# DeltaPavonis/cpp_raytracer

Hardware: AMD Instinct MI355X
Metric: Msamples/sec + achieved HBM GB/s, RTOW final scene at 1/2/4/8 MI355X (higher is better)
Workload: dtype f64; 1 GPU; rtow_final seed 42, 1200x800, 500 spp, max_depth 50 (BASELINE config 2); primitives=485, bvh_nodes=115, partition=whole frame on one GPU

## Files before the change

cpp_raytracer_amd/csrc/crt_device.hip:

```cpp
#include <hip/hip_runtime.h>

#define CRT_HD __host__ __device__ __forceinline__

#include <algorithm>
#include <atomic>
#include <cmath>
#include <cstdio>
#include <cstring>
#include <limits>
#include <string>
#include <mutex>
#include <thread>
#include <type_traits>
#include <vector>

#include "crt_internal.h"
#include "crt_hip_util.h"
#include "crt_rows.h"
#include "crt_ray_class.h"
#include "crt_schlick.h"

#pragma clang fp contract(off)

namespace crt {

namespace dev {

#ifndef CRT_BLOCK
#define CRT_BLOCK 256
#endif
constexpr int kBlock = CRT_BLOCK;
#ifndef CRT_TILE_W
#define CRT_TILE_W 16
#endif
constexpr uint32_t kTileW = CRT_TILE_W, kTileH = 64 / CRT_TILE_W;
constexpr int kManyWaves = 5;
#ifndef CRT_PAIR_WALK
#define CRT_PAIR_WALK 1
#endif
constexpr double kScale = 1 / static_cast<double>(4294967295u - 1);

typedef double Dvec2 __attribute__((ext_vector_type(2)));
typedef uint32_t Uvec4 __attribute__((ext_vector_type(4)));

struct SceneView {
    const DevNode* nodes;
    const DevNodeF* fnodes;
    uint32_t ntop;
    const uint32_t* refs;
    const DevSphere* spheres;
    const DevSpherePair* spair;
    uint32_t spair_lds;
    const uint32_t* sphere_mat;
    const DevQuad* quads;
    const uint32_t* quad_mat;
    const DevMaterial* mats;
    const DevQuadF* quadf;
    const DevMaterial* sphere_mrec;
    const DevMaterial* quad_mrec;
    uint32_t quadf_lds;
    const DevQuadBox* quadbox;
    uint32_t refs_lds, spheres_lds, quads_lds;
    uint32_t inv64_lds;
    unsigned long long* guard;
    const uint16_t* links;
    uint32_t links_lds;
    uint32_t sentinel;
};

struct CamView {
    double o[3], p00[3], pdx[3], pdy[3], ddx[3], ddy[3];
    double defocus_angle;
    double bg[3];
    double t_min;
    double inv_spp;
    uint32_t w, h, spp, max_depth, base_seed;
};

struct Work {
    uint32_t owned_rows;
    uint32_t row_block, tile_count, tile_index;
    uint32_t col0, k0, bw, bh;
    uint32_t tiles_x, tiles_y, tiles;
    uint32_t chunks, chunk_len;
    uint32_t s0;
    uint32_t* queue;
    uint32_t segments;
    uint32_t n_items, bulk_items;
    uint32_t item_chunks, groups, bulk_chunks, tail_chunks;
    uint32_t rb_shift;
    uint32_t lds_nodes, lds_refs, lds_spheres, lds_quads, lds_quadf, lds_stack;
    uint32_t bytes_nodes, bytes_refs, bytes_spheres, bytes_quads, bytes_quadf;
    uint32_t lds_sph64, bytes_sph64;
    uint32_t sphere_only;
    uint32_t exact_slab;
    uint32_t ntop;
    uint32_t sentinel;
    uint32_t lds_cam;
    uint32_t lds_acc;
    uint32_t lds_inv64;
    uint32_t lds_links, bytes_links;
    uint32_t packed;
// ... 93 lines not shown
    h = fma(h, e, h);
    double d = fma(-g, g, x);
    g = fma(d, h, g);
    d = fma(-g, g, x);
    return fma(d, h, g);
}

template <bool FAST>
__device__ __forceinline__ double sqrt_exact(double x) {
    if (FAST) return sqrt_from_rsq(x, __builtin_amdgcn_rsq(x));
    return sqrt(x);
}
__device__ __forceinline__ double recip_core(double s) {
    double y = __builtin_amdgcn_rcp(s);
    y = fma(y, fma(-s, y, 1.0), y);
    y = fma(y, fma(-s, y, 1.0), y);
    return fma(fma(-s, y, 1.0), y, y);
}
template <bool FAST>
__device__ __forceinline__ double recip_exact(double s) {
    if (!FAST) return 1 / s;
    if (__builtin_expect(!(fabs(s) >= 0x1p-500 && fabs(s) <= 0x1p500), 0)) return 1 / s;
    return recip_core(s);
}

template <bool FAST = false>
__device__ __forceinline__ void random_unit_vector(uint32_t& s, double& x, double& y, double& z) {
    double m2;
    do {
        x = rnd_pm1(s);
        y = rnd_pm1(s);
        z = rnd_pm1(s);
        m2 = x * x + y * y + z * z;
    } while (!(m2 < 1));
    double inv = recip_exact<FAST>(sqrt_exact<FAST>(x * x + y * y + z * z));
    x = x * inv;
    y = y * inv;
    z = z * inv;
}

struct NodeRegs {
    double b[6];
    uint32_t index, count, axis, flags;
};

__device__ __forceinline__ NodeRegs load_node(const DevNode* nodes, uint32_t i) {
    const uint4* p = reinterpret_cast<const uint4*>(nodes + i);
    const uint4 q0 = p[0], q1 = p[1], q2 = p[2], q3 = p[3];
    NodeRegs n;
    n.b[0] = __hiloint2double(q0.y, q0.x);
    n.b[1] = __hiloint2double(q0.w, q0.z);
    n.b[2] = __hiloint2double(q1.y, q1.x);
    n.b[3] = __hiloint2double(q1.w, q1.z);
    n.b[4] = __hiloint2double(q2.y, q2.x);
    n.b[5] = __hiloint2double(q2.w, q2.z);
    n.index = q3.x;
    n.count = q3.y;
    n.axis = q3.z;
    n.flags = q3.w;
    return n;
}

__device__ __forceinline__ bool slab(const NodeRegs& n, const double o[3], const double inv[3],
                                     uint32_t neg, double tmin, double tmax) {
    const double bx0 = (neg & 1u) ? n.b[1] : n.b[0], bx1 = (neg & 1u) ? n.b[0] : n.b[1];
    const double by0 = (neg & 2u) ? n.b[3] : n.b[2], by1 = (neg & 2u) ? n.b[2] : n.b[3];
    const double bz0 = (neg & 4u) ? n.b[5] : n.b[4], bz1 = (neg & 4u) ? n.b[4] : n.b[5];
    double xtmin = (bx0 - o[0]) * inv[0];
    double xtmax = (bx1 - o[0]) * inv[0];
    const double ytmin = (by0 - o[1]) * inv[1];
    const double ytmax = (by1 - o[1]) * inv[1];
    const double ztmin = (bz0 - o[2]) * inv[2];
    const double ztmax = (bz1 - o[2]) * inv[2];
    const bool c1 = !(xtmin > ytmax || ytmin > xtmax);
    if (ytmin > xtmin) xtmin = ytmin;
    if (ytmax < xtmax) xtmax = ytmax;
    const bool c2 = !(xtmin > ztmax || ztmin > xtmax);
    if (ztmin > xtmin) xtmin = ztmin;
    if (ztmax < xtmax) xtmax = ztmax;
    return c1 & c2 & (xtmin < tmax) & (xtmax > tmin);
}

template <bool FAST = false>
__device__ __forceinline__ double recip_a(double a) {
    return (a >= 0x1p-500 && a <= 0x1p500) ? (FAST ? recip_core(a) : 1 / a) : __builtin_nan("");
}

__device__ __forceinline__ double div_a(double n, double a, double ia) {
    const double an = fabs(n);
    if (__builtin_expect(!(an >= 0x1p-500 && an <= 0x1p500 && ia == ia), 0)) return n / a;
    double q = n * ia;
    q = fma(fma(-a, q, n), ia, q);
    return fma(fma(-a, q, n), ia, q);
}

__device__ __forceinline__ double lim_tmax(double tmax, double a) { return tmax * a * (1 + 0x1p-30); }
__device__ __forceinline__ double lim_tmin(double tmin, double a) { return tmin * a * (1 - 0x1p-30); }

template <bool COARSE = true>
__device__ __forceinline__ bool hit_sphere(const DevSphere& sp, const double o[3], const double d[3],
                                           double a, double ia, double tmin, double tmax, double lo,
                                           double hi, double& t) {
    double ocx = o[0] - sp.c[0], ocy = o[1] - sp.c[1], ocz = o[2] - sp.c[2];
    double b = d[0] * ocx + d[1] * ocy + d[2] * ocz;
    double c = (ocx * ocx + ocy * ocy + ocz * ocz) - sp.r * sp.r;
    double disc = b * b - a * c;
    if (disc < 0) return false;
    const double rs = __builtin_amdgcn_rsq(disc);
    if (COARSE) {
        const double sqa = disc * rs;
        const double m = (fabs(b) + sqa) * 0x1p-12;
        const bool beyond = (-b - sqa) - m > hi;
        const bool before = (-b + sqa) + m < lo;
        if (beyond || before) return false;
    }
    double sq = sqrt_from_rsq(disc, rs);
    double root = div_a(-b - sq, a, ia);
    if (!(tmin < root && root < tmax)) {
        root = div_a(-b + sq, a, ia);
        if (!(tmin < root && root < tmax)) return false;
    }
    t = root;
    return true;
}

__device__ __forceinline__ float vmin(float a, float b) { float r; asm("v_min_f32 %0, %1, %2" : "=v"(r) : "v"(a), "v"(b)); return r; }
__device__ __forceinline__ float vmax(float a, float b) { float r; asm("v_max_f32 %0, %1, %2" : "=v"(r) : "v"(a), "v"(b)); return r; }
__device__ __forceinline__ float vmin3(float a, float b, float c) {
    float r;
    asm("v_min3_f32 %0, %1, %2, %3" : "=v"(r) : "v"(a), "v"(b), "v"(c));
    return r;
}
__device__ __forceinline__ float vmax_s(float a, float b) { float r; asm("v_max_f32 %0, %2, %1" : "=v"(r) : "v"(a), "s"(b)); return r; }
__device__ __forceinline__ float vmax_abs(float a, float b) {
    float r;
    asm("v_max_f32 %0, |%1|, |%2|" : "=v"(r) : "v"(a), "v"(b));
    return r;
}
__device__ __forceinline__ float vmax3_0(float a, float b) {
    float r;
    asm("v_max3_f32 %0, %1, %2, 0" : "=v"(r) : "v"(a), "v"(b));
    return r;
}
__device__ __forceinline__ float vmax3(float a, float b, float c) {
    float r;
    asm("v_max3_f32 %0, %1, %2, %3" : "=v"(r) : "v"(a), "v"(b), "v"(c));
    return r;
}

struct DevMinMax {
    static __device__ __forceinline__ float min(float a, float b) { return vmin(a, b); }
    static __device__ __forceinline__ float max(float a, float b) { return vmax(a, b); }
    static __device__ __forceinline__ float min3(float a, float b, float c) { return vmin3(a, b, c); }
    static __device__ __forceinline__ float max3(float a, float b, float c) { return vmax3(a, b, c); }
    static __device__ __forceinline__ float max_s(float a, float b) { return vmax_s(a, b); }
    static __device__ __forceinline__ float max_abs(float a, float b) { return vmax_abs(a, b); }
};

typedef float F2 __attribute__((ext_vector_type(2)));
struct LeafRay32 {
    F2 oxy, ozdx, dydz, akap, hilo;
};
__device__ __forceinline__ void leaf_ray32(const double o[3], const double d[3], double a, double tmin,
                                           double tmax, LeafRay32& L) {
    float o32[3];
    double e2 = 0;
#pragma unroll
    for (int k = 0; k < 3; ++k) {
        o32[k] = static_cast<float>(o[k]);
        const double e = o[k] - static_cast<double>(o32[k]);
        e2 = e2 + e * e;
    }
    L.oxy = F2{o32[0], o32[1]};
    L.ozdx = F2{o32[2], static_cast<float>(d[0])};
    L.dydz = F2{static_cast<float>(d[1]), static_cast<float>(d[2])};
    L.akap = F2{static_cast<float>(a), static_cast<float>(e2 * 0x1p22 + 0x1p-50)};
    L.hilo = F2{static_cast<float>(tmax * a * (1 + 0x1p-20)), static_cast<float>(tmin * a * (1 - 0x1p-20))};
}
__device__ __forceinline__ bool leaf_ray32_ok(const double o[3], const double d[3], double a) {
    bool ok = a >= 0x1p-60 && a <= 0x1p60;
#pragma unroll
    for (int k = 0; k < 3; ++k) ok = ok && fabs(o[k]) <= 0x1p30 && fabs(d[k]) <= 0x1p30;
    return ok;
}
__device__ __forceinline__ float vmul_abs(float a, float b) {
    float r;
    asm("v_mul_f32 %0, %1, |%2|" : "=v"(r) : "v"(a), "v"(b));
    return r;
}
__device__ __forceinline__ F2 sub_pL(F2 p, F2 c) {
    F2 r;
    asm("v_pk_add_f32 %0, %1, %2 op_sel_hi:[0,1] neg_lo:[0,1] neg_hi:[0,1]" : "=v"(r) : "v"(p), "v"(c));
    return r;
}
__device__ __forceinline__ F2 sub_pH(F2 p, F2 c) {
    F2 r;
    asm("v_pk_add_f32 %0, %1, %2 op_sel:[1,0] op_sel_hi:[1,1] neg_lo:[0,1] neg_hi:[0,1]" : "=v"(r) : "v"(p), "v"(c));
    return r;
}
__device__ __forceinline__ F2 add_pH(F2 p, F2 c) {
    F2 r;
    asm("v_pk_add_f32 %0, %1, %2 op_sel:[1,0] op_sel_hi:[1,1]" : "=v"(r) : "v"(p), "v"(c));
    return r;
}
__device__ __forceinline__ F2 mul_pL(F2 p, F2 c) {
    F2 r;
    asm("v_pk_mul_f32 %0, %1, %2 op_sel_hi:[0,1]" : "=v"(r) : "v"(p), "v"(c));
    return r;
}
__device__ __forceinline__ F2 mul_pH(F2 p, F2 c) {
    F2 r;
    asm("v_pk_mul_f32 %0, %1, %2 op_sel:[1,0] op_sel_hi:[1,1]" : "=v"(r) : "v"(p), "v"(c));
    return r;
}
__device__ __forceinline__ F2 fma_pL(F2 p, F2 c, F2 e) {
    F2 r;
    asm("v_pk_fma_f32 %0, %1, %2, %3 op_sel_hi:[0,1,1]" : "=v"(r) : "v"(p), "v"(c), "v"(e));
    return r;
}
__device__ __forceinline__ F2 fma_pH(F2 p, F2 c, F2 e) {
    F2 r;
    asm("v_pk_fma_f32 %0, %1, %2, %3 op_sel:[1,0,0] op_sel_hi:[1,1,1]" : "=v"(r) : "v"(p), "v"(c), "v"(e));
    return r;
}
__device__ __forceinline__ F2 nsub_pL(F2 b, F2 p) {
    F2 r;
    asm("v_pk_add_f32 %0, %1, %2 op_sel_hi:[1,0] neg_lo:[1,1] neg_hi:[1,1]" : "=v"(r) : "v"(b), "v"(p));
    return r;
}
__device__ __forceinline__ F2 add_bH(F2 b, F2 p) {
    F2 r;
    asm("v_pk_add_f32 %0, %1, %2 op_sel:[0,1] op_sel_hi:[1,1]" : "=v"(r) : "v"(b), "v"(p));
    return r;
}
typedef float Fvec4 __attribute__((ext_vector_type(4)));
struct PairLines {
    Fvec4 c;
    Fvec4 zr;
};
typedef __attribute__((address_space(3))) const PairLines LdsPair;
typedef __attribute__((address_space(1))) const PairLines GlobalPair;
template <typename P>
__device__ __forceinline__ DevSpherePair pair_at(P p) {
    const Fvec4 c = p->c, zr = p->zr;
    DevSpherePair r;
    r.cx[0] = c.x; r.cx[1] = c.y; r.cy[0] = c.z; r.cy[1] = c.w;
    r.cz[0] = zr.x; r.cz[1] = zr.y; r.r2e[0] = zr.z; r.r2e[1] = zr.w;
    return r;
}
struct SphereLines {
    Dvec2 a, b;
};
typedef __attribute__((address_space(1))) const SphereLines GlobalSphere;
__device__ __forceinline__ DevSphere sphere_global(const DevSphere* p) {
    const GlobalSphere* q = (GlobalSphere*)p;
    const Dvec2 a = q->a, b = q->b;
    DevSphere r;
    r.c[0] = a.x; r.c[1] = a.y; r.c[2] = b.x; r.r = b.y;
    return r;
}
typedef __attribute__((address_space(1))) const Fvec4 GlobalFvec4;
__device__ __forceinline__ DevQuadF quadf_global(const DevQuadF* p) {
    const GlobalFvec4* q = (GlobalFvec4*)p;
    DevQuadF r;
    Fvec4* dst = reinterpret_cast<Fvec4*>(&r);
#pragma unroll
// ... 98 lines not shown
        nrm[0] = nx; nrm[1] = ny; nrm[2] = nz;
        front = true;
    }
    return m;
}

template <typename SE>
struct Stack {
    SE* base;
    uint32_t stride;
    __device__ __forceinline__ void put(int i, uint32_t v) { base[static_cast<size_t>(i) * stride] = static_cast<SE>(v); }
    __device__ __forceinline__ uint32_t get(int i) const { return base[static_cast<size_t>(i) * stride]; }
};

template <typename SE, bool COUNT>
__device__ __forceinline__ bool trace(const SceneView& S, Stack<SE>& st, const double o[3],
                                      const double d[3], double tmin, double& tmax,
                                      uint32_t& hit_ref, LaneCounters& ctr) {
    const double inv[3] = {1 / d[0], 1 / d[1], 1 / d[2]};
    const uint32_t neg = (d[0] < 0 ? 1u : 0u) | (d[1] < 0 ? 2u : 0u) | (d[2] < 0 ? 4u : 0u);
    const double a = d[0] * d[0] + d[1] * d[1] + d[2] * d[2];
    const double ia = recip_a(a), lo = lim_tmin(tmin, a);
    double hi = lim_tmax(tmax, a);
    bool found = false;
    int sp = 0;
    uint32_t cur = 0;
    bool done = false;
    while (!done) {
        uint32_t first = 0, count = 0;
        while (true) {
            const NodeRegs n = load_node(S.nodes, cur);
            if (COUNT) ctr.nodes++;
            const bool enter = slab(n, o, inv, neg, tmin, tmax) | (n.count > 0 && (n.flags & kNodeAlways) != 0);
            if (enter) {
                if (n.count > 0) {
                    first = n.index;
                    count = n.count;
                    break;
                }
                if ((neg >> n.axis) & 1u) {
                    st.put(sp++, n.flags);
                    cur = n.index;
                } else {
                    st.put(sp++, n.index);
                    cur = n.flags;
                }
            } else {
                if (sp == 0) {
                    done = true;
                    break;
                }
                cur = st.get(--sp);
            }
        }
        for (uint32_t i = first; i < first + count; ++i) {
            const uint32_t ref = S.refs[i];
            double t;
            bool h;
            if (ref & kRefQuad) {
                if (COUNT) ctr.quad_tests++;
                h = hit_quad(S.quads[ref & ~kRefQuad], o, d, tmin, tmax, t);
            } else {
                if (COUNT) ctr.sphere_tests++;
                h = hit_sphere(S.spheres[ref], o, d, a, ia, tmin, tmax, lo, hi, t);
            }
            if (h) {
                tmax = t;
                hi = lim_tmax(t, a);
                hit_ref = ref;
                found = true;
            }
        }
        if (count > 0) {
            if (sp == 0) done = true;
            else cur = st.get(--sp);
        }
    }
    return found;
}

enum : uint32_t { kWalk = 0, kLeaf = 1, kDone = 2, kIdle = 3 };

constexpr uint32_t kZeroDir = 8u;

struct Trav {
    float inv32[3], oinv32[3];
    float marg;
    float tmax32;
    double a;
    double tmax;
    uint32_t cur, ref;
    int32_t sp;
    uint32_t first, count;
    uint32_t neg;
    uint32_t state;
    bool found;
};

__device__ __forceinline__ bool finite_nonzero(double x) { return fabs(x) < __builtin_inf() && x != 0; }
__device__ __forceinline__ bool finite(double x) { return fabs(x) < __builtin_inf(); }
__device__ __forceinline__ float tmax_f32(double t) { return static_cast<float>(fmin(t, 0x1p100)); }

__device__ __forceinline__ bool dir_ok(double x) { return fabs(x) >= 0x1p-1000 && fabs(x) <= 0x1p1000; }

__device__ __forceinline__ void trav_init(const double o[3], const double d[3], bool f32_ok, Trav& R) {
    R.a = d[0] * d[0] + d[1] * d[1] + d[2] * d[2];
    R.tmax = __builtin_inf();
    R.tmax32 = 0x1p100f;
    R.cur = 0;
    R.sp = 0;
    R.ref = 0;
    const bool fast = dir_ok(d[0]) && dir_ok(d[1]) && dir_ok(d[2]) &&
                      finite(o[0]) && finite(o[1]) && finite(o[2]);
    R.neg = (d[0] < 0 ? 1u : 0u) | (d[1] < 0 ? 2u : 0u) | (d[2] < 0 ? 4u : 0u) | (fast ? 0u : kZeroDir);
    bool f32 = f32_ok;
    float A = 0;
#pragma unroll
    for (int k = 0; k < 3; ++k) {
        const float d32 = static_cast<float>(d[k]), o32 = static_cast<float>(o[k]);
        R.inv32[k] = __builtin_amdgcn_rcpf(d32);
        R.oinv32[k] = o32 * R.inv32[k];
        A = __builtin_fmaxf(A, __builtin_fabsf(R.oinv32[k]));
        f32 = f32 && __builtin_fabsf(d32) <= 0x1p39f && __builtin_fabsf(d32) >= 0x1p-39f &&
              __builtin_fabsf(o32) <= 0x1p40f;
    }
    R.marg = f32 ? __builtin_fmaxf(A * 0x1p-19f, 0x1p-60f) : __builtin_inff();
    R.state = kWalk;
    R.found = false;
}

typedef __attribute__((address_space(3))) const unsigned char LdsByte;
struct NodeLines {
    Dvec2 b[3];
    Uvec4 meta;
};
template <typename P>
__device__ __forceinline__ void node_lines(P p, NodeLines& n) {
    n.b[0] = p->b[0];
    n.b[1] = p->b[1];
    n.b[2] = p->b[2];
    n.meta = p->meta;
}
typedef __attribute__((address_space(1))) const NodeLines GlobalNode;
__device__ __forceinline__ GlobalNode* node64(const SceneView& S, uint32_t cur) {
    return (GlobalNode*)(S.nodes + (cur >> kNodeFShift));
}

__device__ __forceinline__ bool slab64(GlobalNode* p, const double o[3], const double d[3], double tmin,
                                       double tmax) {
    NodeLines nd;
    node_lines(p, nd);
    double dx = d[0], dy = d[1], dz = d[2];
    asm volatile("" : "+v"(dx), "+v"(dy), "+v"(dz));
    const double inv[3] = {1 / dx, 1 / dy, 1 / dz};
    const Dvec2 bx = nd.b[0], by = nd.b[1], bz = nd.b[2];
    const double x0 = (bx.x - o[0]) * inv[0], x1 = (bx.y - o[0]) * inv[0];
    const double y0 = (by.x - o[1]) * inv[1], y1 = (by.y - o[1]) * inv[1];
    const double z0 = (bz.x - o[2]) * inv[2], z1 = (bz.y - o[2]) * inv[2];
    const double near = fmax(fmax(fmin(x0, x1), fmin(y0, y1)), fmin(z0, z1));
    const double far = fmin(fmin(fmax(x0, x1), fmax(y0, y1)), fmax(z0, z1));
    return (near <= far) & (near < tmax) & (far > tmin);
}

__device__ __forceinline__ bool slab64_inv(GlobalNode* p, const double o[3], uint32_t inv_lds, double tmin,
                                           double tmax) {
    NodeLines nd;
    node_lines(p, nd);
    typedef __attribute__((address_space(3))) const double LdsDoubleC;
    uint32_t t = threadIdx.x;
    asm volatile("" : "+v"(t));
    LdsDoubleC* q = (LdsDoubleC*)static_cast<uintptr_t>(inv_lds + t * 8);
    const double inv[3] = {q[0], q[kBlock], q[2 * kBlock]};
    const Dvec2 bx = nd.b[0], by = nd.b[1], bz = nd.b[2];
    const double x0 = (bx.x - o[0]) * inv[0], x1 = (bx.y - o[0]) * inv[0];
    const double y0 = (by.x - o[1]) * inv[1], y1 = (by.y - o[1]) * inv[1];
    const double z0 = (bz.x - o[2]) * inv[2], z1 = (bz.y - o[2]) * inv[2];
    const double near = fmax(fmax(fmin(x0, x1), fmin(y0, y1)), fmin(z0, z1));
    const double far = fmin(fmin(fmax(x0, x1), fmax(y0, y1)), fmax(z0, z1));
    return (near <= far) & (near < tmax) & (far > tmin);
}

struct NodeF {
    Uvec4 q0;
    Uvec4 q1;
};
typedef __attribute__((address_space(3))) const NodeF LdsNodeF;
typedef __attribute__((address_space(1))) const NodeF GlobalNodeF;
template <bool TOP, bool LS>
__device__ __forceinline__ void fetch_nodef(const SceneView& S, uint32_t cur, Uvec4& q0, Uvec4& q1) {
    if (LS) {
        LdsNodeF* p = (LdsNodeF*)static_cast<uintptr_t>(cur);
        q0 = p->q0;
        q1 = p->q1;
    } else if (TOP) {
        const uint64_t hbm = __ballot(cur >= S.ntop);
        uint64_t save;
        asm volatile(
            "s_and_saveexec_b64 %[save], %[hbm]\n\t"
            "s_cbranch_execz 1f\n\t"
            "global_load_dwordx4 %[q0], %[cur], %[base]\n\t"
            "global_load_dwordx4 %[q1], %[cur], %[base] offset:16\n"
            "1:\n\t"
            "s_andn2_b64 exec, %[save], %[hbm]\n\t"
            "s_cbranch_execz 2f\n\t"
            "ds_read_b128 %[q0], %[cur]\n\t"
            "ds_read_b128 %[q1], %[cur] offset:16\n"
            "2:\n\t"
            "s_mov_b64 exec, %[save]\n\t"
            "s_waitcnt vmcnt(0) lgkmcnt(0)"
            : [q0] "=&v"(q0), [q1] "=&v"(q1), [save] "=&s"(save)
            : [cur] "v"(cur), [hbm] "s"(hbm), [base] "s"(S.fnodes)
            : "memory");
    } else {
        GlobalNodeF* p = (GlobalNodeF*)(reinterpret_cast<const char*>(S.fnodes) + cur);
        q0 = p->q0;
        q1 = p->q1;
    }
}

typedef uint32_t Uvec2 __attribute__((ext_vector_type(2)));
template <bool TOP, bool LS>
__device__ __forceinline__ Uvec2 fetch_nodef_words(const SceneView& S, uint32_t cur) {
    typedef __attribute__((address_space(3))) const Uvec2 LdsU2;
    typedef __attribute__((address_space(1))) const Uvec2 GlobalU2;
    if (LS) return *(LdsU2*)static_cast<uintptr_t>(cur + 24);
    if (!TOP) return *(GlobalU2*)(reinterpret_cast<const char*>(S.fnodes) + cur + 24);
    const uint64_t hbm = __ballot(cur >= S.ntop);
    uint64_t save;
    Uvec2 w;
    asm volatile(
        "s_and_saveexec_b64 %[save], %[hbm]\n\t"
        "s_cbranch_execz 1f\n\t"
        "global_load_dwordx2 %[w], %[cur], %[base] offset:24\n"
        "1:\n\t"
        "s_andn2_b64 exec, %[save], %[hbm]\n\t"
        "s_cbranch_execz 2f\n\t"
        "ds_read_b64 %[w], %[cur] offset:24\n"
        "2:\n\t"
        "s_mov_b64 exec, %[save]\n\t"
        "s_waitcnt vmcnt(0) lgkmcnt(0)"
        : [w] "=&v"(w), [save] "=&s"(save)
        : [cur] "v"(cur), [hbm] "s"(hbm), [base] "s"(S.fnodes)
        : "memory");
    return w;
}

typedef __attribute__((address_space(3))) const uint16_t LdsU16;
__device__ __forceinline__ uint32_t link_at(uint32_t lbase, uint32_t cur) {
    return *(LdsU16*)static_cast<uintptr_t>(lbase + (cur >> 1));
}

template <typename SE, bool COUNT, bool EXACT, bool TOP, bool LS, bool GS, bool SPEC, bool INVL = false, bool G2 = true,
          bool LINK = false>
__device__ __forceinline__ void walk(const SceneView& S, Stack<SE>& st, const double o[3], const double d[3],
                                     double tmin, float tmin32, Trav& R, LaneCounters& ctr) {
    static_assert(!LINK || (LS && !GS && !TOP), "miss links are staged by the LDS-scene instances only");
    const ptrdiff_t stride = LINK ? 0 : static_cast<ptrdiff_t>(st.stride);
    SE* const empty = LINK ? nullptr : st.base - stride;
    SE* tp = LINK ? nullptr : st.base + (static_cast<ptrdiff_t>(R.sp) - 1) * stride;
    const uint32_t lbase = LINK ? S.links_lds + ((R.neg & 7u) << 1) : 0u;
    uint32_t cur = R.cur;
    uint32_t w0, w1;
    bool stop;
    if (EXACT) {
        double dx = d[0], dy = d[1], dz = d[2];
        asm volatile("" : "+v"(dx), "+v"(dy), "+v"(dz));
        const double inv[3] = {1 / dx, 1 / dy, 1 / dz};
        do {
            NodeLines nd;
            node_lines(node64(S, cur), nd);
            const Uvec4 meta = nd.meta;
            const uint32_t top = LINK ? link_at(lbase, cur) : *tp;
            if (COUNT) {
                if (meta.y != kSentinelCount) ctr.nodes++;
                if (wave_leader()) ctr.it_walk++;
            }
            const bool nx = R.neg & 1u, ny = (R.neg >> 1) & 1u, nz = (R.neg >> 2) & 1u;
            const double bx0 = nx ? nd.b[0].y : nd.b[0].x, bx1 = nx ? nd.b[0].x : nd.b[0].y;
            const double by0 = ny ? nd.b[1].y : nd.b[1].x, by1 = ny ? nd.b[1].x : nd.b[1].y;
            const double bz0 = nz ? nd.b[2].y : nd.b[2].x, bz1 = nz ? nd.b[2].x : nd.b[2].y;
            double xtmin = (bx0 - o[0]) * inv[0];
            double xtmax = (bx1 - o[0]) * inv[0];
            const double ytmin = (by0 - o[1]) * inv[1];
            const double ytmax = (by1 - o[1]) * inv[1];
            const double ztmin = (bz0 - o[2]) * inv[2];
            const double ztmax = (bz1 - o[2]) * inv[2];
            const bool c1 = !(xtmin > ytmax || ytmin > xtmax);
            if (ytmin > xtmin) xtmin = ytmin;
            if (ytmax < xtmax) xtmax = ytmax;
            const bool c2 = !(xtmin > ztmax || ztmin > xtmax);
            if (ztmin > xtmin) xtmin = ztmin;
            if (ztmax < xtmax) xtmax = ztmax;
            const bool enter = (c1 & c2 & (xtmin < R.tmax) & (xtmax > tmin)) |
                               (meta.y != 0 && (meta.w & kNodeAlways) != 0) | (meta.y == kSentinelCount);
            const bool inner = enter & (meta.y == 0);
            const bool far_first = (R.neg >> meta.z) & 1u;
            const uint32_t left = meta.w << kNodeFShift, right = meta.x << kNodeFShift;
            if (!LINK) tp[stride] = static_cast<SE>(far_first ? left : right);
            stop = enter ^ inner;
            cur = inner ? (far_first ? right : left) : top;
            if (!LINK) tp += inner ? stride : -stride;
            w0 = meta.x;
            w1 = meta.y == kSentinelCount ? kSentinelW1 : (kLeafFlagF | meta.y);
        } while (!stop);
    } else if (SPEC) {
        bool run = true, nopend = true;
        uint32_t pref = ~0u, pcur = 0;
        do {
            CRT_WD(4, cur, static_cast<uint32_t>(tp - empty));
            if (run) {
                Uvec4 q0, q1;
                fetch_nodef<TOP, LS>(S, cur, q0, q1);
                w0 = q1.z;
                w1 = q1.w;
                const uint32_t top = LINK ? link_at(lbase, cur) : *tp;
                if (COUNT) {
                    if (w1 != kSentinelW1) ctr.nodes++;
                    if (wave_leader()) ctr.it_walk++;
                }
                const float x0 = __builtin_fmaf(__uint_as_float(q0.x), R.inv32[0], -R.oinv32[0]);
                const float x1 = __builtin_fmaf(__uint_as_float(q0.y), R.inv32[0], -R.oinv32[0]);
                const float y0 = __builtin_fmaf(__uint_as_float(q0.z), R.inv32[1], -R.oinv32[1]);
                const float y1 = __builtin_fmaf(__uint_as_float(q0.w), R.inv32[1], -R.oinv32[1]);
                const float z0 = __builtin_fmaf(__uint_as_float(q1.x), R.inv32[2], -R.oinv32[2]);
                const float z1 = __builtin_fmaf(__uint_as_float(q1.y), R.inv32[2], -R.oinv32[2]);
                const float lo = vmax3(vmin(x0, x1), vmin(y0, y1), vmax_s(vmin(z0, z1), tmin32));
                const float hi = vmin3(vmax(x0, x1), vmax(y0, y1), vmin(vmax(z0, z1), R.tmax32));
                const float gap = hi - lo;
                const float th = __builtin_fmaf(vmax_abs(lo, hi), 0x1p-19f, R.marg);
                bool enter = gap > 0.f;
                const bool unc = !(fabsf(gap) > th);
                if (__builtin_expect(__ballot(unc) != 0, 0)) {
                    if (COUNT && wave_leader()) ctr.it_slow++;
                    if (unc) {
                        if (COUNT) ctr.slow_nodes++;
                        enter = INVL ? slab64_inv(node64(S, cur), o, S.inv64_lds, tmin, R.tmax)
                                     : slab64(node64(S, cur), o, d, tmin, R.tmax);
                    }
                }
                const bool inner = enter & (w1 < kLeafFlagF);
                const uint32_t near = w1 | (__builtin_amdgcn_ubfe(R.neg, w0, 1) << kNodeFShift);
                if (!LINK) tp[stride] = static_cast<SE>(near ^ (1u << kNodeFShift));
                const bool reached = enter & !inner;
                const bool park = reached & (!nopend | (!G2 && w1 == kSentinelW1));
                pref = (reached & nopend) ? cur : pref;
                pcur = park ? cur : pcur;
                run = !park;
                cur = inner ? near : top;
                if (!LINK) tp += inner ? stride : -stride;
            }
            nopend = pref == ~0u;
        } while (__ballot(nopend) != 0);
        if (!run) {
            cur = pcur;
            if (!LINK) tp += stride;
        }
        {
            const Uvec2 w = fetch_nodef_words<TOP, LS>(S, pref);
            w0 = w.x;
            w1 = w.y;
        }
        R.state = w1 == kSentinelW1 ? kDone : kLeaf;
        R.first = w0;
        R.count = w1 & ~kLeafFlagF;
        R.cur = cur;
        if (!LINK) R.sp = static_cast<int32_t>(static_cast<uint32_t>(tp - empty)) / static_cast<int32_t>(st.stride);
        return;
    } else {
        do {
            CRT_WD(5, cur, static_cast<uint32_t>(tp - empty));
            Uvec4 q0, q1;
            fetch_nodef<TOP, LS>(S, cur, q0, q1);
            w0 = q1.z;
            w1 = q1.w;
            const uint32_t top = LINK ? link_at(lbase, cur) : *tp;
            if (COUNT) {
                if (w1 != kSentinelW1) ctr.nodes++;
                if (wave_leader()) ctr.it_walk++;
            }
            const float x0 = __builtin_fmaf(__uint_as_float(q0.x), R.inv32[0], -R.oinv32[0]);
            const float x1 = __builtin_fmaf(__uint_as_float(q0.y), R.inv32[0], -R.oinv32[0]);
            const float y0 = __builtin_fmaf(__uint_as_float(q0.z), R.inv32[1], -R.oinv32[1]);
            const float y1 = __builtin_fmaf(__uint_as_float(q0.w), R.inv32[1], -R.oinv32[1]);
            const float z0 = __builtin_fmaf(__uint_as_float(q1.x), R.inv32[2], -R.oinv32[2]);
            const float z1 = __builtin_fmaf(__uint_as_float(q1.y), R.inv32[2], -R.oinv32[2]);
            const float lo = vmax3(vmin(x0, x1), vmin(y0, y1), vmax_s(vmin(z0, z1), tmin32));
            const float hi = vmin3(vmax(x0, x1), vmax(y0, y1), vmin(vmax(z0, z1), R.tmax32));
            const float gap = hi - lo;
            const float th = __builtin_fmaf(vmax_abs(lo, hi), 0x1p-19f, R.marg);
            bool enter = gap > 0.f;
            const bool unc = !(fabsf(gap) > th);
            if (__builtin_expect(__ballot(unc) != 0, 0)) {
                if (COUNT && wave_leader()) ctr.it_slow++;
                if (unc) {
                    if (COUNT) ctr.slow_nodes++;
                    enter = INVL ? slab64_inv(node64(S, cur), o, S.inv64_lds, tmin, R.tmax)
                                 : slab64(node64(S, cur), o, d, tmin, R.tmax);
                }
            }
            const bool inner = enter & (w1 < kLeafFlagF);
            const uint32_t near = w1 | (__builtin_amdgcn_ubfe(R.neg, w0, 1) << kNodeFShift);
            if (!LINK) tp[stride] = static_cast<SE>(near ^ (1u << kNodeFShift));
            stop = enter ^ inner;
            cur = inner ? near : top;
            if (!LINK) tp += inner ? stride : -stride;
        } while (!stop);
    }
    R.state = w1 == kSentinelW1 ? kDone : kLeaf;
    R.first = w0;
    R.count = w1 & ~kLeafFlagF;
    R.cur = cur;
    if (!LINK) R.sp = static_cast<int32_t>(static_cast<uint32_t>(tp - empty)) / static_cast<int32_t>(st.stride);
}


constexpr uint32_t kTokAlone = 1u;

__device__ __forceinline__ uint32_t vsel(uint64_t m, uint32_t a, uint32_t b) {
    uint32_t r;
    asm("v_cndmask_b32_e64 %0, %1, %2, %3" : "=v"(r) : "v"(b), "v"(a), "s"(m));
    return r;
}

template <bool TOP>
__device__ __forceinline__ void fetch_two(const SceneView& S, uint32_t f, uint32_t g, Uvec4& a0, Uvec4& a1, Uvec4& b0,
                                          Uvec4& b1) {
    if (TOP) {
        const uint64_t hbm = __ballot(f >= S.ntop);
        uint64_t save;
        asm volatile(
            "s_and_saveexec_b64 %[save], %[hbm]\n\t"
            "s_cbranch_execz 1f\n\t"
            "global_load_dwordx4 %[a0], %[f], %[base]\n\t"
            "global_load_dwordx4 %[a1], %[f], %[base] offset:16\n\t"
            "global_load_dwordx4 %[b0], %[g], %[base]\n\t"
            "global_load_dwordx4 %[b1], %[g], %[base] offset:16\n"
            "1:\n\t"
            "s_andn2_b64 exec, %[save], %[hbm]\n\t"
            "s_cbranch_execz 2f\n\t"
            "ds_read_b128 %[a0], %[f]\n\t"
            "ds_read_b128 %[a1], %[f] offset:16\n\t"
            "ds_read_b128 %[b0], %[g]\n\t"
            "ds_read_b128 %[b1], %[g] offset:16\n"
            "2:\n\t"
            "s_mov_b64 exec, %[save]\n\t"
            "s_waitcnt vmcnt(0) lgkmcnt(0)"
            : [a0] "=&v"(a0), [a1] "=&v"(a1), [b0] "=&v"(b0), [b1] "=&v"(b1), [save] "=&s"(save)
            : [f] "v"(f), [g] "v"(g), [hbm] "s"(hbm), [base] "s"(S.fnodes)
            : "memory");
    } else {
        GlobalNodeF* qa = (GlobalNodeF*)(reinterpret_cast<const char*>(S.fnodes) + f);
        GlobalNodeF* qb = (GlobalNodeF*)(reinterpret_cast<const char*>(S.fnodes) + g);
        a0 = qa->q0;
        a1 = qa->q1;
        b0 = qb->q0;
        b1 = qb->q1;
    }
}

__device__ __forceinline__ void node_lohi(const Uvec4& q0, const Uvec4& q1, const Trav& R, float tmin32, float& lo,
                                          float& hi) {
    const float x0 = __builtin_fmaf(__uint_as_float(q0.x), R.inv32[0], -R.oinv32[0]);
    const float x1 = __builtin_fmaf(__uint_as_float(q0.y), R.inv32[0], -R.oinv32[0]);
    const float y0 = __builtin_fmaf(__uint_as_float(q0.z), R.inv32[1], -R.oinv32[1]);
    const float y1 = __builtin_fmaf(__uint_as_float(q0.w), R.inv32[1], -R.oinv32[1]);
    const float z0 = __builtin_fmaf(__uint_as_float(q1.x), R.inv32[2], -R.oinv32[2]);
    const float z1 = __builtin_fmaf(__uint_as_float(q1.y), R.inv32[2], -R.oinv32[2]);
    lo = vmax3(vmin(x0, x1), vmin(y0, y1), vmax_s(vmin(z0, z1), tmin32));
    hi = vmin3(vmax(x0, x1), vmax(y0, y1), vmin(vmax(z0, z1), R.tmax32));
}

template <typename SE, bool COUNT, bool TOP, bool INVL>
__device__ __forceinline__ void walk_pairs(const SceneView& S, Stack<SE>& st, const double o[3], const double d[3],
                                           double tmin, float tmin32, Trav& R, LaneCounters& ctr) {
    const ptrdiff_t stride = static_cast<ptrdiff_t>(st.stride);
    SE* const empty = st.base - stride;
    SE* tp = st.base + (static_cast<ptrdiff_t>(R.sp) - 1) * stride;
    uint32_t cur = R.cur;
    uint32_t run = 1;
    uint32_t pref = ~0u;
    uint64_t nop = __ballot(true);
    do {
        CRT_WD(7, cur, static_cast<uint32_t>(tp - empty));
        if (run) {
            const uint32_t f = cur & ~kTokAlone, g = f ^ 32u;
            Uvec4 a0, a1, b0, b1;
            fetch_two<TOP>(S, f, g, a0, a1, b0, b1);
            const uint32_t top = *tp;
            float lo1, hi1, lo2, hi2;
            node_lohi(a0, a1, R, tmin32, lo1, hi1);
            node_lohi(b0, b1, R, tmin32, lo2, hi2);
            const float g1 = hi1 - lo1, g2 = hi2 - lo2;
            const float t1 = __builtin_fmaf(vmax_abs(lo1, hi1), 0x1p-19f, R.marg);
            const float t2 = __builtin_fmaf(vmax_abs(lo2, hi2), 0x1p-19f, R.marg);
            const uint64_t two = __ballot(cur == f);
            uint64_t e1 = __ballot(g1 > 0.f), e2 = __ballot(g2 > 0.f) & two;
            const uint64_t u1 = __ballot(!(fabsf(g1) > t1)), u2 = two & __ballot(!(fabsf(g2) > t2));
            if (COUNT) {
                if (a1.w != kSentinelW1) ctr.nodes++;
                ctr.nodes += cur == f ? 1 : 0;
                if (wave_leader()) ctr.it_walk++;
            }
            if (__builtin_expect((u1 | u2) != 0, 0)) {
                if (COUNT && wave_leader()) ctr.it_slow++;
                const uint64_t me = 1ull << (threadIdx.x & 63);
                bool f1 = false, f2 = false;
                if (u1 & me) {
                    if (COUNT) ctr.slow_nodes++;
                    f1 = INVL ? slab64_inv(node64(S, f), o, S.inv64_lds, tmin, R.tmax) : slab64(node64(S, f), o, d, tmin, R.tmax);
                }
                if (u2 & me) {
                    if (COUNT) ctr.slow_nodes++;
                    f2 = INVL ? slab64_inv(node64(S, g), o, S.inv64_lds, tmin, R.tmax) : slab64(node64(S, g), o, d, tmin, R.tmax);
                }
                e1 = (e1 & ~u1) | __ballot(f1);
                e2 = (e2 & ~u2) | __ballot(f2);
            }
            const uint64_t i1 = __ballot(a1.w < kLeafFlagF), i2 = __ballot(b1.w < kLeafFlagF);
            const uint64_t both = e1 & e2, any = e1 | e2;
            const uint64_t xi = (e1 & i1) | (~e1 & i2);
            const uint64_t leaf = any & ~xi;
            const uint64_t park = leaf & ~nop;
            const uint64_t dp = (any & xi) | park;
            const uint32_t tok1 = vsel(i1, (__builtin_amdgcn_ubfe(R.neg, a1.z, 1) << kNodeFShift) | a1.w, cur | kTokAlone);
            const uint32_t tok2 = vsel(i2, (__builtin_amdgcn_ubfe(R.neg, b1.z, 1) << kNodeFShift) | b1.w, g | kTokAlone);
            const uint32_t tx = vsel(e1, tok1, tok2);
            pref = vsel(leaf & nop, tx, pref);
            tp[stride] = static_cast<SE>(tok2);
            cur = vsel(dp, tx, vsel(both, tok2, top));
            tp += static_cast<int32_t>(vsel(dp & both, 1u, vsel(~dp & ~both, ~0u, 0u))) * stride;
            run = vsel(park, 0u, 1u);
        }
        nop = __ballot(pref == ~0u);
    } while (nop != 0);
    {
        const Uvec2 w = fetch_nodef_words<TOP, false>(S, pref & ~kTokAlone);
        R.state = w.y == kSentinelW1 ? kDone : kLeaf;
        R.first = w.x;
        R.count = w.y & ~kLeafFlagF;
    }
    R.cur = cur;
    R.sp = static_cast<int32_t>(static_cast<uint32_t>(tp - empty)) / static_cast<int32_t>(st.stride);
}

template <typename SE, bool COUNT, bool TOP, bool LS, bool FAST = false, bool QONLY = false, bool LINK = false>
__device__ __forceinline__ void leaf_step(const SceneView& S, Stack<SE>& st, const double o[3],
                                              const double d[3], double tmin, float tmin32, bool sphere_only, bool pairs,
                                              bool qfilter, bool qflat, Trav& R, LaneCounters& ctr) {
    const uint2 range = make_uint2(R.first, R.count);
    const uint32_t end = range.x + range.y;
    const double ia = recip_a<FAST>(R.a), lo = lim_tmin(tmin, R.a);
    double hi = lim_tmax(R.tmax, R.a);
    if (!QONLY && pairs && range.y <= 32 && leaf_ray32_ok(o, d, R.a)) {
        LeafRay32 L;
        leaf_ray32(o, d, R.a, tmin, R.tmax, L);
        uint32_t cand = 0;
        const uint32_t nbits = (range.y + 1) & ~1u;
        if constexpr (LS) {
            for (uint32_t i = 0; i < range.y; i += 2) {
                if (COUNT) {
                    ctr.sphere_tests += i + 1 < range.y ? 2 : 1;
                    if (wave_leader()) ctr.it_leaf += 2;
                }
                cand = sphere_pair_candidates(cand, pair_at((LdsPair*)static_cast<uintptr_t>(S.spair_lds + ((range.x + i) << 5))), L);
            }
        } else {
            for (uint32_t i = 0; i < range.y; i += 2) {
                if (COUNT) {
                    ctr.sphere_tests += i + 1 < range.y ? 2 : 1;
                    if (wave_leader()) ctr.it_leaf += 2;
                }
                cand = sphere_pair_candidates(cand, pair_at((GlobalPair*)(S.spair + range.x + i)), L);
            }
        }
        cand &= ~(range.y & 1u);
        while (cand) {
            CRT_WD(6, cand, range.y);
            if (COUNT) {
                ctr.cand++;
                if (wave_leader()) ctr.it_cand++;
            }
            const uint32_t b = 31 - __builtin_clz(cand);
            cand ^= 1u << b;
            const uint32_t i = range.x + (nbits - 1 - b);
            double t;
            if (hit_sphere<false>(sphere_at<LS>(S, i), o, d, R.a, ia, tmin, R.tmax, lo, hi, t)) {
                R.tmax = t;
                R.tmax32 = tmax_f32(t);
                hi = lim_tmax(t, R.a);
                R.ref = i;
                R.found = true;
            }
        }
    } else if (LS && qfilter && qflat && range.y <= 32) {
        uint32_t cand = 0;
        const uint32_t base = S.quadf_lds + (range.x << 5);
        const uint32_t g = lds_u32(base + 28);
        const uint32_t e0 = g & 0xffu, e1 = e0 + ((g >> 8) & 0xffu);
        uint32_t i = 0;
        const auto filter = [&](auto axis) {
            if (COUNT) {
                ctr.quad_tests++;
                if (wave_leader()) ctr.it_leaf++;
            }
            LdsNodeF* p = (LdsNodeF*)static_cast<uintptr_t>(base + (i << 5));
            const Uvec4 q0 = p->q0, q1 = p->q1;
            const float b[6] = {__uint_as_float(q0.x), __uint_as_float(q0.y), __uint_as_float(q0.z),
                                __uint_as_float(q0.w), __uint_as_float(q1.x), __uint_as_float(q1.y)};
            cand |= static_cast<uint32_t>(flat_axis_candidate<decltype(axis)::value, DevMinMax>(b, R.inv32, R.oinv32, tmin32, R.tmax32, R.marg)) << q1.z;
        };
        for (; i < e0; ++i) filter(std::integral_constant<int, 0>{});
        for (; i < e1; ++i) filter(std::integral_constant<int, 1>{});
        for (; i < range.y; ++i) filter(std::integral_constant<int, 2>{});
        while (cand) {
            CRT_WD(6, cand, range.y);
            if (COUNT) {
                ctr.cand++;
                if (wave_leader()) ctr.it_cand++;
            }
            const uint32_t i = range.x + static_cast<uint32_t>(__builtin_ctz(cand));
            cand &= cand - 1;
            double t;
            if (hit_quad(lds_rec<DevQuad>(S.quads_lds + (i << 7)), o, d, tmin, R.tmax, t)) {
                R.tmax = t;
                R.tmax32 = tmax_f32(t);
                R.ref = kRefQuad | i;
                R.found = true;
            }
        }
    } else if (LS && qfilter && !qflat && range.y <= 32 && quad_ray32_ok(o, d)) {
        QuadRay32 L;
        quad_ray32(o, d, tmin, R.tmax, L);
        uint32_t cand = 0;
        for (uint32_t i = 0; i < range.y; ++i) {
            if (COUNT) {
                ctr.quad_tests++;
// ... 2940 lines not shown
```

Baseline: 6901 Msamples/s.

## Hoist per-ray range gates into one cheap check and rework SPEC walk with wave masks

Replaces the per-call double-precision range checks (direction/origin finiteness, leaf32 eligibility, reciprocal range) with a single cheap f32 gate at traversal init. The detailed checks run only when some lane in the wave fails it, and their outcomes are cached as flag bits in R.neg. The speculative BVH walk loop is also restructured to track pending and parked lanes with ballot masks and exec-masked cndmask selects instead of per-lane booleans, which reduces VALU work and divergence in the inner loop. The risk is subtle correctness issues from the hand-written inline asm using exec and vcc, plus a change in loop exit semantics.

```diff
diff --git a/cpp_raytracer_amd/csrc/crt_device.hip b/cpp_raytracer_amd/csrc/crt_device.hip
--- a/cpp_raytracer_amd/csrc/crt_device.hip
+++ b/cpp_raytracer_amd/csrc/crt_device.hip
@@ -18,6 +18,7 @@
 #include "crt_hip_util.h"
 #include "crt_rows.h"
 #include "crt_ray_class.h"
+#include "crt_ray_gate.h"
 #include "crt_schlick.h"
 
 #pragma clang fp contract(off)
@@ -277,9 +278,11 @@
 }
 
 template <bool FAST = false>
-__device__ __forceinline__ double recip_a(double a) {
-    return (a >= 0x1p-500 && a <= 0x1p500) ? (FAST ? recip_core(a) : 1 / a) : __builtin_nan("");
-}
+__device__ __forceinline__ double recip_a(double a, bool in_range) {
+    return in_range ? (FAST ? recip_core(a) : 1 / a) : __builtin_nan("");
+}
+template <bool FAST = false>
+__device__ __forceinline__ double recip_a(double a) { return recip_a<FAST>(a, gate_recip(a)); }
 
 __device__ __forceinline__ double div_a(double n, double a, double ia) {
     const double an = fabs(n);
@@ -319,6 +322,33 @@
     return true;
 }
 
+__device__ __forceinline__ uint32_t vsel(uint64_t m, uint32_t a, uint32_t b) {
+    uint32_t r;
+    asm("v_cndmask_b32_e64 %0, %1, %2, %3" : "=v"(r) : "v"(b), "v"(a), "s"(m));
+    return r;
+}
+
+__device__ __forceinline__ uint32_t vsel_top_on(uint64_t on, uint64_t m, uint32_t a, uint16_t top, uint32_t keep) {
+    uint64_t save;
+    asm("s_and_saveexec_b64 %[save], %[on]\n\t"
+        "s_mov_b64 vcc, %[m]\n\t"
+        "v_cndmask_b32_sdwa %[r], %[b], %[a], vcc dst_sel:DWORD dst_unused:UNUSED_PAD src0_sel:WORD_0 src1_sel:DWORD\n\t"
+        "s_mov_b64 exec, %[save]"
+        : [r] "+v"(keep), [save] "=&s"(save)
+        : [a] "v"(a), [b] "v"(__builtin_bit_cast(_Float16, top)), [m] "s"(m), [on] "s"(on)
+        : "vcc", "scc");
+    return keep;
+}
+__device__ __forceinline__ uint32_t vsel_top_on(uint64_t on, uint64_t m, uint32_t a, uint32_t top, uint32_t keep) {
+    uint64_t save;
+    asm("s_and_saveexec_b64 %[save], %[on]\n\t"
+        "v_cndmask_b32_e64 %[r], %[b], %[a], %[m]\n\t"
+        "s_mov_b64 exec, %[save]"
+        : [r] "+v"(keep), [save] "=&s"(save)
+        : [a] "v"(a), [b] "v"(top), [m] "s"(m), [on] "s"(on)
+        : "scc");
+    return keep;
+}
 __device__ __forceinline__ float vmin(float a, float b) { float r; asm("v_min_f32 %0, %1, %2" : "=v"(r) : "v"(a), "v"(b)); return r; }
 __device__ __forceinline__ float vmax(float a, float b) { float r; asm("v_max_f32 %0, %1, %2" : "=v"(r) : "v"(a), "v"(b)); return r; }
 __device__ __forceinline__ float vmin3(float a, float b, float c) {
@@ -371,12 +401,6 @@
     L.dydz = F2{static_cast<float>(d[1]), static_cast<float>(d[2])};
     L.akap = F2{static_cast<float>(a), static_cast<float>(e2 * 0x1p22 + 0x1p-50)};
     L.hilo = F2{static_cast<float>(tmax * a * (1 + 0x1p-20)), static_cast<float>(tmin * a * (1 - 0x1p-20))};
-}
-__device__ __forceinline__ bool leaf_ray32_ok(const double o[3], const double d[3], double a) {
-    bool ok = a >= 0x1p-60 && a <= 0x1p60;
-#pragma unroll
-    for (int k = 0; k < 3; ++k) ok = ok && fabs(o[k]) <= 0x1p30 && fabs(d[k]) <= 0x1p30;
-    return ok;
 }
 __device__ __forceinline__ float vmul_abs(float a, float b) {
     float r;
@@ -641,6 +665,7 @@
 enum : uint32_t { kWalk = 0, kLeaf = 1, kDone = 2, kIdle = 3 };
 
 constexpr uint32_t kZeroDir = 8u;
+constexpr uint32_t kNoLeaf32 = 16u, kNoRecip = 32u;
 
 struct Trav {
     float inv32[3], oinv32[3];
@@ -660,8 +685,6 @@
 __device__ __forceinline__ bool finite(double x) { return fabs(x) < __builtin_inf(); }
 __device__ __forceinline__ float tmax_f32(double t) { return static_cast<float>(fmin(t, 0x1p100)); }
 
-__device__ __forceinline__ bool dir_ok(double x) { return fabs(x) >= 0x1p-1000 && fabs(x) <= 0x1p1000; }
-
 __device__ __forceinline__ void trav_init(const double o[3], const double d[3], bool f32_ok, Trav& R) {
     R.a = d[0] * d[0] + d[1] * d[1] + d[2] * d[2];
     R.tmax = __builtin_inf();
@@ -669,19 +692,22 @@
     R.cur = 0;
     R.sp = 0;
     R.ref = 0;
-    const bool fast = dir_ok(d[0]) && dir_ok(d[1]) && dir_ok(d[2]) &&
-                      finite(o[0]) && finite(o[1]) && finite(o[2]);
-    R.neg = (d[0] < 0 ? 1u : 0u) | (d[1] < 0 ? 2u : 0u) | (d[2] < 0 ? 4u : 0u) | (fast ? 0u : kZeroDir);
-    bool f32 = f32_ok;
-    float A = 0;
+    float d32[3], o32[3];
 #pragma unroll
     for (int k = 0; k < 3; ++k) {
-        const float d32 = static_cast<float>(d[k]), o32 = static_cast<float>(o[k]);
-        R.inv32[k] = __builtin_amdgcn_rcpf(d32);
-        R.oinv32[k] = o32 * R.inv32[k];
-        A = __builtin_fmaxf(A, __builtin_fabsf(R.oinv32[k]));
-        f32 = f32 && __builtin_fabsf(d32) <= 0x1p39f && __builtin_fabsf(d32) >= 0x1p-39f &&
-              __builtin_fabsf(o32) <= 0x1p40f;
+        d32[k] = static_cast<float>(d[k]);
+        o32[k] = static_cast<float>(o[k]);
+        R.inv32[k] = __builtin_amdgcn_rcpf(d32[k]);
+        R.oinv32[k] = o32[k] * R.inv32[k];
+    }
+    const float A = __builtin_fmaxf(__builtin_fmaxf(__builtin_fabsf(R.oinv32[0]), __builtin_fabsf(R.oinv32[1])),
+                                    __builtin_fabsf(R.oinv32[2]));
+    R.neg = (d[0] < 0 ? 1u : 0u) | (d[1] < 0 ? 2u : 0u) | (d[2] < 0 ? 4u : 0u);
+    bool f32 = f32_ok;
+    if (__builtin_expect(__ballot(!ray_gate(o32, d32)) != 0, 0)) {
+        f32 = f32 && gate_walk_f32(o32, d32);
+        R.neg |= (gate_walk_plain(o, d) ? 0u : kZeroDir) | (gate_leaf32(o, d, R.a) ? 0u : kNoLeaf32) |
+                 (gate_recip(R.a) ? 0u : kNoRecip);
     }
     R.marg = f32 ? __builtin_fmaxf(A * 0x1p-19f, 0x1p-60f) : __builtin_inff();
     R.state = kWalk;
@@ -805,9 +831,10 @@
 }
 
 typedef __attribute__((address_space(3))) const uint16_t LdsU16;
-__device__ __forceinline__ uint32_t link_at(uint32_t lbase, uint32_t cur) {
+__device__ __forceinline__ uint16_t link16_at(uint32_t lbase, uint32_t cur) {
     return *(LdsU16*)static_cast<uintptr_t>(lbase + (cur >> 1));
 }
+__device__ __forceinline__ uint32_t link_at(uint32_t lbase, uint32_t cur) { return link16_at(lbase, cur); }
 
 template <typename SE, bool COUNT, bool EXACT, bool TOP, bool LS, bool GS, bool SPEC, bool INVL = false, bool G2 = true,
           bool LINK = false>
@@ -823,7 +850,8 @@
     bool stop;
     if (EXACT) {
         double dx = d[0], dy = d[1], dz = d[2];
-        asm volatile("" : "+v"(dx), "+v"(dy), "+v"(dz));
+        uint32_t neg = R.neg;
+        asm volatile("" : "+v"(dx), "+v"(dy), "+v"(dz), "+v"(neg));
         const double inv[3] = {1 / dx, 1 / dy, 1 / dz};
         do {
             NodeLines nd;
@@ -834,7 +862,7 @@
                 if (meta.y != kSentinelCount) ctr.nodes++;
                 if (wave_leader()) ctr.it_walk++;
             }
-            const bool nx = R.neg & 1u, ny = (R.neg >> 1) & 1u, nz = (R.neg >> 2) & 1u;
+            const bool nx = neg & 1u, ny = (neg >> 1) & 1u, nz = (neg >> 2) & 1u;
             const double bx0 = nx ? nd.b[0].y : nd.b[0].x, bx1 = nx ? nd.b[0].x : nd.b[0].y;
             const double by0 = ny ? nd.b[1].y : nd.b[1].x, by1 = ny ? nd.b[1].x : nd.b[1].y;
             const double bz0 = nz ? nd.b[2].y : nd.b[2].x, bz1 = nz ? nd.b[2].x : nd.b[2].y;
@@ -853,7 +881,7 @@
             const bool enter = (c1 & c2 & (xtmin < R.tmax) & (xtmax > tmin)) |
                                (meta.y != 0 && (meta.w & kNodeAlways) != 0) | (meta.y == kSentinelCount);
             const bool inner = enter & (meta.y == 0);
-            const bool far_first = (R.neg >> meta.z) & 1u;
+            const bool far_first = (neg >> meta.z) & 1u;
             const uint32_t left = meta.w << kNodeFShift, right = meta.x << kNodeFShift;
             if (!LINK) tp[stride] = static_cast<SE>(far_first ? left : right);
             stop = enter ^ inner;
@@ -863,16 +891,20 @@
             w1 = meta.y == kSentinelCount ? kSentinelW1 : (kLeafFlagF | meta.y);
         } while (!stop);
     } else if (SPEC) {
-        bool run = true, nopend = true;
-        uint32_t pref = ~0u, pcur = 0;
-        do {
+        bool rec = false;
+        uint64_t nop = __ballot(true);
+        uint32_t pref = 0;
+        for (;;) {
             CRT_WD(4, cur, static_cast<uint32_t>(tp - empty));
-            if (run) {
+            {
                 Uvec4 q0, q1;
                 fetch_nodef<TOP, LS>(S, cur, q0, q1);
                 w0 = q1.z;
                 w1 = q1.w;
-                const uint32_t top = LINK ? link_at(lbase, cur) : *tp;
+                const auto top = [&] {
+                    if constexpr (LINK) return link16_at(lbase, cur);
+                    else return *tp;
+                }();
                 if (COUNT) {
                     if (w1 != kSentinelW1) ctr.nodes++;
                     if (wave_leader()) ctr.it_walk++;
@@ -887,32 +919,34 @@
                 const float hi = vmin3(vmax(x0, x1), vmax(y0, y1), vmin(vmax(z0, z1), R.tmax32));
                 const float gap = hi - lo;
                 const float th = __builtin_fmaf(vmax_abs(lo, hi), 0x1p-19f, R.marg);
-                bool enter = gap > 0.f;
+                float dec = gap;
                 const bool unc = !(fabsf(gap) > th);
                 if (__builtin_expect(__ballot(unc) != 0, 0)) {
                     if (COUNT && wave_leader()) ctr.it_slow++;
                     if (unc) {
                         if (COUNT) ctr.slow_nodes++;
-                        enter = INVL ? slab64_inv(node64(S, cur), o, S.inv64_lds, tmin, R.tmax)
-                                     : slab64(node64(S, cur), o, d, tmin, R.tmax);
+                        dec = (INVL ? slab64_inv(node64(S, cur), o, S.inv64_lds, tmin, R.tmax)
+                                    : slab64(node64(S, cur), o, d, tmin, R.tmax)) ? 1.f : -1.f;
                     }
                 }
-                const bool inner = enter & (w1 < kLeafFlagF);
+                const bool enter = dec > 0.f, leaf = w1 >= kLeafFlagF;
+                const uint64_t em = __ballot(enter), lm = __ballot(leaf);
+                const uint64_t im = em & ~lm;
+                const uint64_t rm = em & lm;
                 const uint32_t near = w1 | (__builtin_amdgcn_ubfe(R.neg, w0, 1) << kNodeFShift);
                 if (!LINK) tp[stride] = static_cast<SE>(near ^ (1u << kNodeFShift));
-                const bool reached = enter & !inner;
-                const bool park = reached & (!nopend | (!G2 && w1 == kSentinelW1));
-                pref = (reached & nopend) ? cur : pref;
-                pcur = park ? cur : pcur;
-                run = !park;
-                cur = inner ? near : top;
-                if (!LINK) tp += inner ? stride : -stride;
-            }
-            nopend = pref == ~0u;
-        } while (__ballot(nopend) != 0);
-        if (!run) {
-            cur = pcur;
-            if (!LINK) tp += stride;
+                const bool reached = enter && leaf;
+                const bool park = reached && (rec || (!G2 && w1 == kSentinelW1));
+                const uint64_t pm = rm & (G2 ? ~nop : (~nop | __ballot(w1 == kSentinelW1)));
+                pref = vsel(rm & nop, cur, pref);
+                nop &= ~rm;
+                rec = rec || reached;
+                const uint64_t on = __ballot(true) & ~pm;
+                cur = vsel_top_on(on, im, near, top, cur);
+                if (!LINK) tp += static_cast<int32_t>(vsel(im & on, static_cast<uint32_t>(stride), vsel(on, static_cast<uint32_t>(-stride), 0u)));
+                if (park) break;
+            }
+            if (nop == 0) break;
         }
         {
             const Uvec2 w = fetch_nodef_words<TOP, LS>(S, pref);
@@ -974,12 +1008,6 @@
 
 
 constexpr uint32_t kTokAlone = 1u;
-
-__device__ __forceinline__ uint32_t vsel(uint64_t m, uint32_t a, uint32_t b) {
-    uint32_t r;
-    asm("v_cndmask_b32_e64 %0, %1, %2, %3" : "=v"(r) : "v"(b), "v"(a), "s"(m));
-    return r;
-}
 
 template <bool TOP>
 __device__ __forceinline__ void fetch_two(const SceneView& S, uint32_t f, uint32_t g, Uvec4& a0, Uvec4& a1, Uvec4& b0,
@@ -1108,9 +1136,9 @@
                                               bool qfilter, bool qflat, Trav& R, LaneCounters& ctr) {
     const uint2 range = make_uint2(R.first, R.count);
     const uint32_t end = range.x + range.y;
-    const double ia = recip_a<FAST>(R.a), lo = lim_tmin(tmin, R.a);
+    const double ia = recip_a<FAST>(R.a, !(R.neg & kNoRecip)), lo = lim_tmin(tmin, R.a);
     double hi = lim_tmax(R.tmax, R.a);
-    if (!QONLY && pairs && range.y <= 32 && leaf_ray32_ok(o, d, R.a)) {
+    if (!QONLY && pairs && range.y <= 32 && !(R.neg & kNoLeaf32)) {
         LeafRay32 L;
         leaf_ray32(o, d, R.a, tmin, R.tmax, L);
         uint32_t cand = 0;
diff --git a/cpp_raytracer_amd/csrc/crt_ray_gate.h b/cpp_raytracer_amd/csrc/crt_ray_gate.h
--- /dev/null
+++ b/cpp_raytracer_amd/csrc/crt_ray_gate.h
@@ -0,0 +1,43 @@
+#pragma once
+
+#ifndef CRT_HD
+#define CRT_HD inline
+#endif
+
+namespace crt {
+
+CRT_HD bool gate_dir_ok(double x) { return __builtin_fabs(x) >= 0x1p-1000 && __builtin_fabs(x) <= 0x1p1000; }
+CRT_HD bool gate_finite(double x) { return __builtin_fabs(x) < __builtin_inf(); }
+
+CRT_HD bool gate_walk_plain(const double o[3], const double d[3]) {
+    return gate_dir_ok(d[0]) && gate_dir_ok(d[1]) && gate_dir_ok(d[2]) &&
+           gate_finite(o[0]) && gate_finite(o[1]) && gate_finite(o[2]);
+}
+
+CRT_HD bool gate_walk_f32(const float o32[3], const float d32[3]) {
+    bool ok = true;
+    for (int k = 0; k < 3; ++k)
+        ok = ok && __builtin_fabsf(d32[k]) <= 0x1p39f && __builtin_fabsf(d32[k]) >= 0x1p-39f &&
+             __builtin_fabsf(o32[k]) <= 0x1p40f;
+    return ok;
+}
+
+CRT_HD bool gate_leaf32(const double o[3], const double d[3], double a) {
+    bool ok = a >= 0x1p-60 && a <= 0x1p60;
+    for (int k = 0; k < 3; ++k) ok = ok && __builtin_fabs(o[k]) <= 0x1p30 && __builtin_fabs(d[k]) <= 0x1p30;
+    return ok;
+}
+
+CRT_HD bool gate_recip(double a) { return a >= 0x1p-500 && a <= 0x1p500; }
+
+constexpr float kGateMax = 0x1p29f, kGateMinDir = 0x1p-29f;
+
+CRT_HD bool ray_gate(const float o32[3], const float d32[3]) {
+    const float sd = (__builtin_fabsf(d32[0]) + __builtin_fabsf(d32[1])) + __builtin_fabsf(d32[2]);
+    const float so = (__builtin_fabsf(o32[0]) + __builtin_fabsf(o32[1])) + __builtin_fabsf(o32[2]);
+    const float dmin = __builtin_fminf(__builtin_fminf(__builtin_fabsf(d32[0]), __builtin_fabsf(d32[1])),
+                                       __builtin_fabsf(d32[2]));
+    return sd <= kGateMax && so <= kGateMax && dmin >= kGateMinDir;
+}
+
+}
```

Result: faster. 7008 Msamples/s (median of 6 runs) (+1.5%).
